# ishine/tts-max

Hardware: AMD Instinct MI355X
Metric: audio-codes/sec + RTF@24kHz, TTS-1 bs=1/32, at 1/2/4/8 MI355X (higher is better)
Workload: dtype bf16; 1 GPU; tts1 bf16 bs=1/GPU: prompt 202 tokens (150 codes), 500 greedy codes, codec codec-24k on 650 codes; model=TTS-1 (Llama-3.2-1B dims, V=193856, tied) + xcodec2-style codec codec-24k, global_batch=1, seq_len=702, parallelism=dp1

## Files before the change

### tts-max_amd/csrc/lm_attn.hip

```cpp
#include <stdexcept>

#include "hip_common.h"
#include "lm_kernels.h"
#include "lm_attn_core.h"

namespace tts {

template <int D>
TTS_DEV float rope_at(const bf16_t* v, int d, const bf16_t* cosr, const bf16_t* sinr) {
  constexpr int H2 = D / 2;
  return rope_elem(v[d], v[d < H2 ? d + H2 : d - H2], d < H2, bf2f(cosr[d]), bf2f(sinr[d]));
}

template <int D>
__global__ __launch_bounds__(256) void rope_append_kernel(AttnArgs a) {
  constexpr int VLD = 8 * D + 8;
  __shared__ __attribute__((aligned(16))) bf16_t vs[16 * VLD];
  const int HD = a.H * D, KD = a.KVH * D;
  if ((int)blockIdx.x < a.rows) {
    const int row = blockIdx.x;
    const int slot = a.row_slot[row], pos = a.row_pos[row];
    const bf16_t* base = a.qkv + (size_t)row * a.ld_qkv;
    const bf16_t* cosr = a.rope_cos + (size_t)pos * D;
    const bf16_t* sinr = a.rope_sin + (size_t)pos * D;
    for (int i = threadIdx.x; i < HD + KD; i += blockDim.x) {
      if (i < HD) {
        const int h = i / D, d = i % D;
        a.q_rot[(size_t)row * HD + i] = f2bf(rope_at<D>(base + h * D, d, cosr, sinr));
      } else {
        const int j = i - HD, h = j / D, d = j % D;
        a.kcache[(((size_t)slot * a.KVH + h) * a.max_seq + pos) * D + d] = f2bf(rope_at<D>(base + HD + h * D, d, cosr, sinr));
      }
    }
    return;
  }
  const int4 blk = a.blocks[blockIdx.x - a.rows];
  const int r0 = blk.x, nr = blk.y, slot = blk.z, p0 = blk.w;
  for (int e = threadIdx.x; e < nr * (KD / 8); e += blockDim.x) {
    const int rr = e / (KD / 8), c = e - rr * (KD / 8);
    *(u32x4_t*)(vs + rr * VLD + c * 8) = *(const u32x4_t*)(a.qkv + (size_t)(r0 + rr) * a.ld_qkv + HD + KD + c * 8);
  }
  __syncthreads();
  for (int e = threadIdx.x; e < KD * 16; e += blockDim.x) {
    const int j = e >> 4, pl = e & 15, h = j / D, d = j % D;
    if (pl < nr)
      a.vtcache[((size_t)slot * a.KVH + h) * D * a.max_seq + vt_off(a.max_seq, d, p0 + pl)] = vs[pl * VLD + j];
  }
}

template <int D>
__global__ __launch_bounds__(dec_nw<D>() * 64) void attn_decode_kernel(AttnArgs a) {
  constexpr int PW = dec_pw<D>(), NW = dec_nw<D>();
  using C = DecShape<D, PW>;
  __shared__ __attribute__((aligned(16))) float qs[DEC_G * D];
  __shared__ __attribute__((aligned(16))) bf16_t knew[D];
  __shared__ __attribute__((aligned(16))) bf16_t vnew[D];
  __shared__ __attribute__((aligned(16))) float red[dec_red_floats<D, NW>()];
  const int row = blockIdx.x / a.KVH, kvh = blockIdx.x % a.KVH;
  const int slot = a.row_slot[row], pos = a.row_pos[row], ctx = pos + 1;
  const int tid = threadIdx.x, lane = tid & 63;
  const int wave = __builtin_amdgcn_readfirstlane(tid >> 6);
  const size_t kvbase = ((size_t)slot * a.KVH + kvh) * a.max_seq * D;
  const bf16_t* kc = a.kcache + kvbase;
  const bf16_t* vtc = a.vtcache + kvbase;
  unsigned long long* stp = a.stamps ? a.stamps + 16384 + (size_t)blockIdx.x * 8 : nullptr;
  TTS_STAMP(stp, 0);
  u32x4_t kf[C::MT][C::KS], vf[C::PS][C::DT];
  if (wave * PW < ctx) {
    dec_load_k<D, PW, D == 64>(kc, wave * PW, ctx, lane, kf);
    dec_load_v<D, PW, D == 64>(vtc, a.max_seq, wave * PW, lane, vf);
  }
  const bf16_t* qrow = a.qkv + (size_t)row * a.ld_qkv;
  const bf16_t* cosr = a.rope_cos + (size_t)pos * D;
  const bf16_t* sinr = a.rope_sin + (size_t)pos * D;
  __shared__ __attribute__((aligned(16))) bf16_t raw[DEC_G * D + 2 * D];
  const bf16_t* qsrc = qrow + kvh * DEC_G * D;
  const bf16_t* ksrc = qrow + a.H * D + kvh * D;
  const bf16_t* vsrc = qrow + a.H * D + a.KVH * D + kvh * D;
  if (a.qkv_part) {
    for (int i = tid; i < DEC_G * D + 2 * D; i += NW * 64) {
      const int col = i < DEC_G * D ? kvh * DEC_G * D + i
                    : (i < DEC_G * D + D ? a.H * D + kvh * D + i - DEC_G * D
                                         : a.H * D + a.KVH * D + kvh * D + i - DEC_G * D - D);
      float v = 0.f;
      for (int sl = 0; sl < a.qkv_nsl; ++sl) v += a.qkv_part[((size_t)sl * a.rows + row) * a.ld_qkv + col];
      raw[i] = f2bf(v);
    }
    lds_barrier();
    qsrc = raw;
    ksrc = raw + DEC_G * D;
    vsrc = raw + DEC_G * D + D;
  }
  for (int i = tid; i < DEC_G * D + D; i += NW * 64) {
    if (i < DEC_G * D) {
      const int g = i / D, d = i % D;
      qs[i] = rope_at<D>(qsrc + g * D, d, cosr, sinr);
    } else {
      const int d = i - DEC_G * D;
      knew[d] = f2bf(rope_at<D>(ksrc, d, cosr, sinr));
      vnew[d] = vsrc[d];
    }
  }
  lds_barrier();
  TTS_STAMP(stp, 2);
  dec_attend<D, PW, NW, D == 64>(kc, vtc, a.max_seq, ctx, a.scale, qs, knew, vnew, red, kf, vf,
                              a.out + (size_t)row * a.H * D + kvh * DEC_G * D);
  TTS_STAMP(stp, 3);
  if (tid < D) {
    a.kcache[kvbase + (size_t)pos * D + tid] = knew[tid];
    a.vtcache[kvbase + vt_off(a.max_seq, tid, pos)] = vnew[tid];
  }
}

void launch_attn_decode_step(const AttnArgs& a, hipStream_t s) {
  if (dry_record(a.D == 64 ? "attn_decode_kernel<64>" : "attn_decode_kernel<128>")) return;
  const dim3 grid(a.rows * a.KVH);
  if (a.D == 64) hipLaunchKernelGGL((attn_decode_kernel<64>), grid, dim3(dec_nw<64>() * 64), 0, s, a);
  else hipLaunchKernelGGL((attn_decode_kernel<128>), grid, dim3(dec_nw<128>() * 64), 0, s, a);
}

template <int D>
__global__ __launch_bounds__(256) void attn_prefill_kernel(AttnArgs a) {
  using C = DecShape<D, 32>;
  const int4 blk = a.blocks[blockIdx.x / a.KVH];
  const int kvh = blockIdx.x % a.KVH;
  const int row0 = blk.x, nrows = blk.y, slot = blk.z, pos0 = blk.w;
  const int tid = threadIdx.x, lane = tid & 63;
  const int h = kvh * DEC_G + __builtin_amdgcn_readfirstlane(tid >> 6);
  const int c = lane & 15, g = lane >> 4;
  const int qpos = pos0 + c;
  const int qrow = row0 + min(c, nrows - 1);
  const size_t kvbase = ((size_t)slot * a.KVH + kvh) * a.max_seq * D;
  const bf16_t* kc = a.kcache + kvbase;
  const bf16_t* vtc = a.vtcache + kvbase;
  const int kend = pos0 + nrows;
  const int nkb = (kend + 31) / 32;
  bf16x8_t qb[C::KS];
#pragma unroll
  for (int ks = 0; ks < C::KS; ++ks)
    qb[ks] = __builtin_bit_cast(bf16x8_t, *(const u32x4_t*)(a.q_rot + (size_t)qrow * a.H * D + h * D + 32 * ks + 8 * g));
  auto scores = [&](int kb, f32x4_t (&s)[2]) {
    u32x4_t kf[2][C::KS];
#pragma unroll
    for (int mt = 0; mt < 2; ++mt) {
      const int p = min(dec_pos(kb * 32, mt, c), kend - 1);
#pragma unroll
      for (int ks = 0; ks < C::KS; ++ks) kf[mt][ks] = *(const u32x4_t*)(kc + (size_t)p * D + 32 * ks + 8 * g);
    }
#pragma unroll
    for (int mt = 0; mt < 2; ++mt) {
      f32x4_t acc = {0.f, 0.f, 0.f, 0.f};
#pragma unroll
      for (int ks = 0; ks < C::KS; ++ks)
        acc = __builtin_amdgcn_mfma_f32_16x16x32_bf16(__builtin_bit_cast(bf16x8_t, kf[mt][ks]), qb[ks], acc, 0, 0, 0);
#pragma unroll
      for (int r = 0; r < 4; ++r) acc[r] = (dec_pos(kb * 32, mt, 4 * g + r) <= qpos) ? acc[r] * a.scale : -INFINITY;
      s[mt] = acc;
    }
  };
  float mx = -INFINITY;
  for (int kb = 0; kb < nkb; ++kb) {
    f32x4_t s[2];
    scores(kb, s);
#pragma unroll
    for (int mt = 0; mt < 2; ++mt)
#pragma unroll
      for (int r = 0; r < 4; ++r) mx = fmaxf(mx, s[mt][r]);
  }
  mx = fmaxf(mx, __shfl_xor(mx, 16, 64));
  mx = fmaxf(mx, __shfl_xor(mx, 32, 64));
  float lsum = 0.f;
  f32x4_t o[C::DT];
#pragma unroll
  for (int dt = 0; dt < C::DT; ++dt) o[dt] = f32x4_t{0.f, 0.f, 0.f, 0.f};
  for (int kb = 0; kb < nkb; ++kb) {
    u32x4_t vf[1][C::DT];
    const int p0 = kb * 32 + 8 * g;
#pragma unroll
    for (int dt = 0; dt < C::DT; ++dt) vf[0][dt] = *(const u32x4_t*)(vtc + vt_off(a.max_seq, 16 * dt + c, p0));
// ... 35 lines not shown
```

### tts-max_amd/csrc/lm_attn_core.h

```cpp
#pragma once
#include "hip_common.h"

namespace tts {

template <int D, int PW>
struct DecShape {
  static constexpr int MT = PW / 16;
  static constexpr int KS = D / 32;
  static constexpr int PS = PW / 32;
  static constexpr int DT = D / 16;
};

constexpr int DEC_G = 4;
constexpr int DEC_NW = 16;
template <int D> constexpr int dec_nw() { return 16; }
template <int D> constexpr int dec_pw() { return D == 64 ? 64 : 32; }

TTS_DEV int vt_off(int S, int d, int p) {
  return (((d >> 4) * (S >> 5) + (p >> 5)) * 16 + (d & 15)) * 32 + (p & 31);
}

TTS_DEV int dec_pos(int base, int mt, int row) {
  return base + 32 * (mt >> 1) + 8 * (row >> 2) + 4 * (mt & 1) + (row & 3);
}

template <int D, int PW, bool O32 = false>
TTS_DEV void dec_load_k(const bf16_t* kc, int base, int ctx, int lane,
                        u32x4_t (&kf)[DecShape<D, PW>::MT][DecShape<D, PW>::KS]) {
  using C = DecShape<D, PW>;
  const int c = lane & 15, g = lane >> 4;
#pragma unroll
  for (int mt = 0; mt < C::MT; ++mt) {
    const int p = min(dec_pos(base, mt, c), ctx - 1);
#pragma unroll
    for (int ks = 0; ks < C::KS; ++ks)
      kf[mt][ks] = O32 ? *(const u32x4_t*)(kc + (p * D + 32 * ks + 8 * g))
                       : *(const u32x4_t*)(kc + (size_t)p * D + 32 * ks + 8 * g);
  }
}
template <int D, int PW, bool O32 = false>
TTS_DEV void dec_load_v(const bf16_t* vtc, int S, int base, int lane,
                        u32x4_t (&vf)[DecShape<D, PW>::PS][DecShape<D, PW>::DT]) {
  using C = DecShape<D, PW>;
  const int c = lane & 15, g = lane >> 4;
#pragma unroll
  for (int ps = 0; ps < C::PS; ++ps) {
    const int pb = min((base >> 5) + ps, (S >> 5) - 1);
    const int o0 = (pb * 16 + c) * 32 + 8 * g;
#pragma unroll
    for (int dt = 0; dt < C::DT; ++dt)
      vf[ps][dt] = O32 ? *(const u32x4_t*)(vtc + (o0 + dt * 16 * S)) : *(const u32x4_t*)(vtc + o0 + (size_t)dt * 16 * S);
  }
}

TTS_DEV uint32_t bits_sel(uint32_t mask, uint32_t a, uint32_t b) { return (a & mask) | (b & ~mask); }
template <int D, int PW>
TTS_DEV void dec_patch_k(int base, int ctx, int lane, const bf16_t* knew,
                         u32x4_t (&kf)[DecShape<D, PW>::MT][DecShape<D, PW>::KS]) {
  using C = DecShape<D, PW>;
  const int c = lane & 15, g = lane >> 4, pn = ctx - 1;
  u32x4_t kn[C::KS];
#pragma unroll
  for (int ks = 0; ks < C::KS; ++ks) kn[ks] = *(const u32x4_t*)(knew + 32 * ks + 8 * g);
#pragma unroll
  for (int mt = 0; mt < C::MT; ++mt) {
    const uint32_t m = dec_pos(base, mt, c) == pn ? 0xffffffffu : 0u;
#pragma unroll
    for (int ks = 0; ks < C::KS; ++ks)
#pragma unroll
      for (int q = 0; q < 4; ++q) kf[mt][ks][q] = bits_sel(m, kn[ks][q], kf[mt][ks][q]);
  }
}
template <int D, int PW>
TTS_DEV void dec_patch_v(int base, int ctx, int lane, const bf16_t* vnew,
                         u32x4_t (&vf)[DecShape<D, PW>::PS][DecShape<D, PW>::DT]) {
  using C = DecShape<D, PW>;
  const int c = lane & 15, g = lane >> 4, pn = ctx - 1;
  uint32_t vn[C::DT];
#pragma unroll
  for (int dt = 0; dt < C::DT; ++dt) vn[dt] = vnew[16 * dt + c];
#pragma unroll
  for (int ps = 0; ps < C::PS; ++ps) {
    const int p0 = base + 32 * ps + 8 * g;
    uint32_t keep[4], put[4];
#pragma unroll
    for (int e2 = 0; e2 < 4; ++e2) {
      const int pl = p0 + 2 * e2, ph = pl + 1;
      keep[e2] = (pl < pn ? 0x0000ffffu : 0u) | (ph < pn ? 0xffff0000u : 0u);
      put[e2] = (pl == pn ? 0x0000ffffu : 0u) | (ph == pn ? 0xffff0000u : 0u);
    }
#pragma unroll
    for (int dt = 0; dt < C::DT; ++dt) {
      const uint32_t nv = vn[dt] | (vn[dt] << 16);
#pragma unroll
      for (int e2 = 0; e2 < 4; ++e2) vf[ps][dt][e2] = (vf[ps][dt][e2] & keep[e2]) | (nv & put[e2]);
    }
  }
}

template <int D>
TTS_DEV bf16x8_t dec_qfrag(const float* qs, int lane, int ks) {
  const int h = (lane & 15) & 3, g = lane >> 4;
  const float4 a = *(const float4*)(qs + h * D + 32 * ks + 8 * g);
  const float4 b = *(const float4*)(qs + h * D + 32 * ks + 8 * g + 4);
  const u32x4_t w = {pack_bf2(a.x, a.y), pack_bf2(a.z, a.w), pack_bf2(b.x, b.y), pack_bf2(b.z, b.w)};
  return __builtin_bit_cast(bf16x8_t, w);
}

template <int D, int PW>
TTS_DEV void dec_scores(const u32x4_t (&kf)[DecShape<D, PW>::MT][DecShape<D, PW>::KS], const float* qs,
                        int base, int ctx, float scale, int lane, f32x4_t (&s)[DecShape<D, PW>::MT]) {
  using C = DecShape<D, PW>;
  const int g = lane >> 4;
#pragma unroll
  for (int mt = 0; mt < C::MT; ++mt) s[mt] = f32x4_t{0.f, 0.f, 0.f, 0.f};
#pragma unroll
  for (int ks = 0; ks < C::KS; ++ks) {
    const bf16x8_t qb = dec_qfrag<D>(qs, lane, ks);
#pragma unroll
    for (int mt = 0; mt < C::MT; ++mt)
      s[mt] = __builtin_amdgcn_mfma_f32_16x16x32_bf16(__builtin_bit_cast(bf16x8_t, kf[mt][ks]), qb, s[mt], 0, 0, 0);
  }
#pragma unroll
  for (int mt = 0; mt < C::MT; ++mt)
#pragma unroll
    for (int r = 0; r < 4; ++r) s[mt][r] = (dec_pos(base, mt, 4 * g + r) < ctx) ? s[mt][r] * scale : -INFINITY;
}

template <int D, int PW>
TTS_DEV void dec_pv(float M, float& lsum, f32x4_t (&s)[DecShape<D, PW>::MT],
                    const u32x4_t (&vf)[DecShape<D, PW>::PS][DecShape<D, PW>::DT], f32x4_t (&o)[DecShape<D, PW>::DT]) {
  using C = DecShape<D, PW>;
#pragma unroll
  for (int mt = 0; mt < C::MT; ++mt)
#pragma unroll
    for (int r = 0; r < 4; ++r) {
      const float p = __builtin_amdgcn_exp2f((s[mt][r] - M) * 1.44269504088896341f);
      lsum += p;
      s[mt][r] = p;
    }
#pragma unroll
  for (int ps = 0; ps < C::PS; ++ps) {
    const u32x4_t pw = {pack_bf2(s[2 * ps][0], s[2 * ps][1]), pack_bf2(s[2 * ps][2], s[2 * ps][3]),
                        pack_bf2(s[2 * ps + 1][0], s[2 * ps + 1][1]), pack_bf2(s[2 * ps + 1][2], s[2 * ps + 1][3])};
    const bf16x8_t pb = __builtin_bit_cast(bf16x8_t, pw);
#pragma unroll
    for (int dt = 0; dt < C::DT; ++dt)
      o[dt] = __builtin_amdgcn_mfma_f32_16x16x32_bf16(__builtin_bit_cast(bf16x8_t, vf[ps][dt]), pb, o[dt], 0, 0, 0);
  }
}

template <int D, int NW>
constexpr int dec_red_floats() { return NW * DEC_G * 2 + NW * DEC_G * D; }

template <int D, int PW, int NW, class Bar, bool O32 = false>
TTS_DEV void dec_attend_w(const bf16_t* kc, const bf16_t* vtc, int S, int ctx, float scale, const float* qs,
                          const bf16_t* knew, const bf16_t* vnew, float* red,
                          u32x4_t (&kf0)[DecShape<D, PW>::MT][DecShape<D, PW>::KS],
                          u32x4_t (&vf0)[DecShape<D, PW>::PS][DecShape<D, PW>::DT], bf16_t* out, int wave,
                          int tid, Bar bar, unsigned long long* stp = nullptr, uint64_t* gout = nullptr,
                          uint32_t gtag = 0) {
  using C = DecShape<D, PW>;
  const int lane = tid & 63;
  const int c = lane & 15, g = lane >> 4;
  const int npass = (ctx + NW * PW - 1) / (NW * PW);
  float* mred = red;
  float* lred = red + NW * DEC_G;
  float* ored = lred + NW * DEC_G;
  const int base0 = wave * PW;

  f32x4_t s0[C::MT];
  float mx = -INFINITY;
  if (base0 < ctx) {
    dec_patch_k<D, PW>(base0, ctx, lane, knew, kf0);
    dec_patch_v<D, PW>(base0, ctx, lane, vnew, vf0);
    dec_scores<D, PW>(kf0, qs, base0, ctx, scale, lane, s0);
#pragma unroll
    for (int mt = 0; mt < C::MT; ++mt)
#pragma unroll
      for (int r = 0; r < 4; ++r) mx = fmaxf(mx, s0[mt][r]);
  }
  for (int ps = 1; ps < npass; ++ps) {
    const int base = (ps * NW + wave) * PW;
    if (base >= ctx) break;
    u32x4_t kf[C::MT][C::KS];
    dec_load_k<D, PW, O32>(kc, base, ctx, lane, kf);
    dec_patch_k<D, PW>(base, ctx, lane, knew, kf);
    f32x4_t s[C::MT];
    dec_scores<D, PW>(kf, qs, base, ctx, scale, lane, s);
#pragma unroll
    for (int mt = 0; mt < C::MT; ++mt)
#pragma unroll
      for (int r = 0; r < 4; ++r) mx = fmaxf(mx, s[mt][r]);
  }
  mx = fmaxf(mx, __shfl_xor(mx, 16, 64));
  mx = fmaxf(mx, __shfl_xor(mx, 32, 64));
  if (lane < DEC_G) mred[wave * DEC_G + lane] = mx;
  bar();
  TTS_STAMP(stp, 5);
  float M = -INFINITY;
#pragma unroll
  for (int w = 0; w < NW; ++w) M = fmaxf(M, mred[w * DEC_G + (c & 3)]);

  float lsum = 0.f;
  f32x4_t o[C::DT];
#pragma unroll
  for (int dt = 0; dt < C::DT; ++dt) o[dt] = f32x4_t{0.f, 0.f, 0.f, 0.f};
  if (base0 < ctx) dec_pv<D, PW>(M, lsum, s0, vf0, o);
  for (int ps = 1; ps < npass; ++ps) {
    const int base = (ps * NW + wave) * PW;
    if (base >= ctx) break;
    u32x4_t kf[C::MT][C::KS], vf[C::PS][C::DT];
    dec_load_v<D, PW, O32>(vtc, S, base, lane, vf);
    dec_load_k<D, PW, O32>(kc, base, ctx, lane, kf);
    dec_patch_k<D, PW>(base, ctx, lane, knew, kf);
    f32x4_t s[C::MT];
    dec_scores<D, PW>(kf, qs, base, ctx, scale, lane, s);
    dec_patch_v<D, PW>(base, ctx, lane, vnew, vf);
    dec_pv<D, PW>(M, lsum, s, vf, o);
  }
  lsum += __shfl_xor(lsum, 16, 64);
  lsum += __shfl_xor(lsum, 32, 64);
  if (c < DEC_G) {
#pragma unroll
    for (int dt = 0; dt < C::DT; ++dt)
      *(float4*)(ored + (wave * DEC_G + c) * D + 16 * dt + 4 * g) = make_float4(o[dt][0], o[dt][1], o[dt][2], o[dt][3]);
    if (g == 0) lred[wave * DEC_G + c] = lsum;
  }
  bar();
  TTS_STAMP(stp, 6);
  bf16_t gob = 0;
  for (int i = tid; i < DEC_G * D; i += NW * 64) {
    const int h = i / D, d = i - h * D;
    float v[NW];
#pragma unroll
    for (int w = 0; w < NW; ++w) v[w] = lred[w * DEC_G + h];
    float O = 0.f, L = 0.f;
#pragma unroll
    for (int w = 0; w < NW; ++w) L += v[w];
#pragma unroll
    for (int w = 0; w < NW; ++w) v[w] = ored[(w * DEC_G + h) * D + d];
#pragma unroll
    for (int w = 0; w < NW; ++w) O += v[w];
    const bf16_t ob = f2bf(O / L);
    out[h * D + d] = ob;
    if (gout) gob = ob;
  }
  if (gout) {
    bar();
    if (tid < DEC_G * D) ((bf16_t*)ored)[tid] = gob;
    bar();
    if (tid < DEC_G * D / 2)
      __hip_atomic_store(gout + tid, ((uint64_t)gtag << 32) | ((const uint32_t*)ored)[tid], __ATOMIC_RELAXED,
                         __HIP_MEMORY_SCOPE_AGENT);
  }
}

template <int D, int PW, int NW, bool O32 = false>
TTS_DEV void dec_attend(const bf16_t* kc, const bf16_t* vtc, int S, int ctx, float scale, const float* qs,
                        const bf16_t* knew, const bf16_t* vnew, float* red,
                        u32x4_t (&kf0)[DecShape<D, PW>::MT][DecShape<D, PW>::KS],
                        u32x4_t (&vf0)[DecShape<D, PW>::PS][DecShape<D, PW>::DT], bf16_t* out,
                        unsigned long long* stp = nullptr, uint64_t* gout = nullptr, uint32_t gtag = 0) {
  auto bar = [] { lds_barrier(); };
  dec_attend_w<D, PW, NW, decltype(bar), O32>(kc, vtc, S, ctx, scale, qs, knew, vnew, red, kf0, vf0, out,
                          __builtin_amdgcn_readfirstlane(threadIdx.x >> 6), threadIdx.x, bar, stp, gout, gtag);
}

TTS_DEV float rope_elem(bf16_t x, bf16_t xr, bool lower_half, float c, float sn) {
  const float rot = lower_half ? -bf2f(xr) : bf2f(xr);
  return rbf(rbf(bf2f(x) * c) + rbf(rot * sn));
}

}
```

### tts-max_amd/csrc/lm_gemm_kernel.h

```cpp
#pragma once
#include <algorithm>
#include <cstdio>
#include <stdexcept>
#include <type_traits>

#include "hip_common.h"
#include "lm_kernels.h"
#include "lm_attn_core.h"

namespace tts {

constexpr int wgemm_ea(int waves) { return waves >= 16 ? 1 : (waves >= 8 ? 2 : 4); }
__host__ __device__ inline int wgemm_red_floats(int waves, int ksplit, int ng, int mt, int M, int Kl) {
  const int upw = waves / ksplit;
  int r = upw * (ksplit - 1) * ng * mt * 4 * 64;
  r = r > upw * mt * 16 * 2 ? r : upw * mt * 16 * 2;
  const int segs = (M * (Kl / 8) + 63) / 64;
  r = r > segs ? r : segs;
  r = r > Kl / 2 ? r : Kl / 2;
  return r + 64;
}

constexpr int wgemm_fattn_d(int ku) { return ku == 2 ? 64 : 128; }
template <int D>
constexpr size_t fattn_lds_bytes() {
  return (size_t)DEC_G * D * 4 + (DEC_G * D / 2 + D) * 4 + 2 * D * 2 + (size_t)dec_red_floats<D, DEC_NW>() * 4;
}
template <typename Poll>
TTS_DEV bool fattn_wait(Poll ready, int* err, int spins, bool report) {
  for (int n = 1; !ready(); ++n) {
    if (n > spins) {
      if (report) __hip_atomic_store(err, 1, __ATOMIC_RELAXED, __HIP_MEMORY_SCOPE_AGENT);
      return false;
    }
    if ((n & 511) == 0 && __hip_atomic_load(err, __ATOMIC_RELAXED, __HIP_MEMORY_SCOPE_AGENT)) return false;
    __builtin_amdgcn_s_sleep(1);
  }
  return true;
}

template <int NT, int D>
TTS_DEV void fattn_consumer(const WgemmArgs& wa, char* smem, int b) {
  static_assert(NT == DEC_NW * 64, "the fused attention runs on 16-wave workgroups");
  constexpr int PW = dec_pw<D>(), G = DEC_G, H2 = D / 2;
  using C = DecShape<D, PW>;
  const AttnArgs& a = wa.fa;
  float* qs = (float*)smem;
  uint32_t* raw = (uint32_t*)(qs + G * D);
  const bf16_t* rawb = (const bf16_t*)raw;
  bf16_t* knew = (bf16_t*)(raw + G * D / 2 + D);
  bf16_t* vnew = knew + D;
  float* red = (float*)(vnew + D);
  const int tid = threadIdx.x, lane = tid & 63;
  const int wave = __builtin_amdgcn_readfirstlane(tid >> 6);
  const int row = b / a.KVH, kvh = b % a.KVH;
  const int slot = a.row_slot[row], pos = a.row_pos[row], ctx = pos + 1;
  const size_t kvbase = ((size_t)slot * a.KVH + kvh) * a.max_seq * D;
  const bf16_t* kc = a.kcache + kvbase;
  const bf16_t* vtc = a.vtcache + kvbase;
  unsigned long long* stp = wa.stamps ? wa.stamps + (size_t)blockIdx.x * 32 : nullptr;
  TTS_STAMP(stp, 0);
  u32x4_t kf[C::MT][C::KS], vf[C::PS][C::DT];
  if (wave * PW < ctx) {
    dec_load_k<D, PW>(kc, wave * PW, ctx, lane, kf);
    dec_load_v<D, PW>(vtc, a.max_seq, wave * PW, lane, vf);
  }
  const int qd = tid % D;
  const float qc = bf2f(a.rope_cos[(size_t)pos * D + qd]), qsn = bf2f(a.rope_sin[(size_t)pos * D + qd]);

  const uint32_t tag = ((uint32_t)pos << 6) | (uint32_t)wa.fattn_layer;
  const int nq = G * D / 2, ngr = nq + D;
  if (tid < ngr) {
    int col;
    if (tid < nq) col = kvh * G * D + 2 * tid;
    else if (tid < nq + D / 2) col = a.H * D + kvh * D + 2 * (tid - nq);
    else col = a.H * D + a.KVH * D + kvh * D + 2 * (tid - nq - D / 2);
    const uint64_t* gp = wa.gran + (size_t)row * (a.ld_qkv / 2) + col / 2;
    uint64_t v;
    fattn_wait([&] {
      v = __hip_atomic_load(gp, __ATOMIC_RELAXED, __HIP_MEMORY_SCOPE_AGENT);
      return (uint32_t)(v >> 32) == tag;
    }, wa.fattn_err, wa.fattn_spins, true);
    raw[tid] = (uint32_t)v;
  }
  lds_barrier();
  TTS_STAMP(stp, 1);
  if (tid < G * D) {
    const int g = tid / D;
    qs[tid] = rope_elem(rawb[tid], rawb[g * D + (qd < H2 ? qd + H2 : qd - H2)], qd < H2, qc, qsn);
  } else if (tid < G * D + D) {
    const int d = tid - G * D;
    knew[d] = f2bf(rope_elem(rawb[G * D + d], rawb[G * D + (d < H2 ? d + H2 : d - H2)], d < H2, qc, qsn));
    vnew[d] = rawb[G * D + D + d];
  }
  lds_barrier();
  TTS_STAMP(stp, 2);
  dec_attend<D, PW, DEC_NW>(kc, vtc, a.max_seq, ctx, a.scale, qs, knew, vnew, red, kf, vf,
                            a.out + (size_t)row * a.H * D + kvh * G * D, stp,
                            wa.fo_units ? wa.gran + (size_t)wa.M * (wa.N / 2) + (size_t)row * (a.H * D / 2) + kvh * G * D / 2
                                        : nullptr,
                            tag);
  TTS_STAMP(stp, 3);
  if (tid < D) {
    a.kcache[kvbase + (size_t)pos * D + tid] = knew[tid];
    a.vtcache[kvbase + vt_off(a.max_seq, tid, pos)] = vnew[tid];
  }
}

TTS_DEV bf16x8_t as_bf16x8(u32x4_t v) { return __builtin_bit_cast(bf16x8_t, v); }

template <int KU, int KSPLIT, int R>
TTS_DEV void fused_oproj(const WgemmArgs& a, bf16_t* xs, float* red, int wave, int lane, uint32_t tag, int u) {
  const int kpart = wave % KSPLIT;
  const int nr = min(a.fo_ur, a.fo_units);
  u32x4_t wr[R][KU];
#pragma unroll
  for (int st = 0; st < R; ++st)
#pragma unroll
    for (int kk = 0; kk < KU; ++kk)
      wr[st][kk] = __builtin_nontemporal_load((const u32x4_t*)a.fo_w +
                                              ((((long long)st * nr + u) * KSPLIT + kpart) * KU + kk) * 64 + lane);
  const bf16_t rr = a.fo_resid[u * 16 + (lane & 15)];
  const uint64_t* g = a.gran + a.N / 2 + kpart * 64 + lane;
  uint64_t v;
  fattn_wait([&] {
    v = __hip_atomic_load(g, __ATOMIC_RELAXED, __HIP_MEMORY_SCOPE_AGENT);
    return (bool)__all((uint32_t)(v >> 32) == tag);
  }, a.fattn_err, a.fattn_spins, lane == 0);
  *(uint32_t*)(xs + kpart * 128 + 2 * lane) = (uint32_t)v;
  asm volatile("s_waitcnt lgkmcnt(0)" ::: "memory");
  f32x4_t acc = {0.f, 0.f, 0.f, 0.f};
  const int akoff = 8 * (lane >> 4);
#pragma unroll
  for (int st = 0; st < R; ++st)
#pragma unroll
    for (int kk = 0; kk < KU; ++kk) {
      const int k = ((kpart * R + st) * KU + kk) * 32 + akoff;
      const u32x4_t av = *(const u32x4_t*)(xs + k);
      acc = __builtin_amdgcn_mfma_f32_16x16x32_bf16(as_bf16x8(av), as_bf16x8(wr[st][kk]), acc, 0, 0, 0);
    }
  if (kpart > 0) *(f32x4_t*)(red + ((size_t)(kpart - 1) * 64 + lane) * 4) = acc;
  lds_barrier();
  if (kpart == 0) {
    constexpr int HB = 8;
#pragma unroll
    for (int p0 = 1; p0 < KSPLIT; p0 += HB) {
      f32x4_t pv[HB];
#pragma unroll
      for (int j = 0; j < HB; ++j)
        if (p0 + j < KSPLIT) pv[j] = *(const f32x4_t*)(red + ((size_t)(p0 + j - 1) * 64 + lane) * 4);
#pragma unroll
      for (int j = 0; j < HB; ++j)
        if (p0 + j < KSPLIT) acc += pv[j];
    }
    if (lane < 16) a.fo_resid[u * 16 + lane] = f2bf(bf2f(rr) + rbf(acc[0]));
  }
}

template <int KU, int KSPLIT, int R>
TTS_DEV void fused_oproj_rows(const WgemmArgs& a, bf16_t* xs, float* red, int wave, int lane, int u) {
  const int M = a.M, HD = a.fa.H * a.fa.D, ldxs = HD + 8, hid = a.fo_units * 16;
  unsigned long long* stp = a.stamps ? a.stamps + (size_t)blockIdx.x * 32 : nullptr;
  TTS_STAMP(stp, 0);
  const int kpart = wave % KSPLIT;
  const int nr = min(a.fo_ur, a.fo_units);
  const int KTc = (HD >> 5) / a.fo_kc, kt_pc = KTc / KSPLIT, Sc = kt_pc / KU;
  auto ktile = [&](int st, int kk) {
    const int ch = st / Sc;
    return ch * KTc + kpart * kt_pc + (st - ch * Sc) * KU + kk;
  };
  u32x4_t wr[R][KU];
#pragma unroll
  for (int st = 0; st < R; ++st)
#pragma unroll
    for (int kk = 0; kk < KU; ++kk)
      wr[st][kk] = __builtin_nontemporal_load((const u32x4_t*)a.fo_w +
                                              ((((long long)st * nr + u) * KSPLIT + kpart) * KU + kk) * 64 + lane);
  bf16_t rr[4];
#pragma unroll
  for (int r = 0; r < 4; ++r) rr[r] = a.fo_resid[(size_t)min(4 * (lane >> 4) + r, M - 1) * hid + u * 16 + (lane & 15)];
// ... 743 lines not shown
```

### tts-max_amd/csrc/lm_head_screen.hip

```cpp
#include <math.h>

#include "hip_common.h"
#include "lm_kernels.h"

namespace tts {

typedef __attribute__((ext_vector_type(4))) int i32x4_t;

namespace {

constexpr int kScrWaves = 4;
constexpr int kScrKU = 8;
constexpr int kScrR = 2;

TTS_DEV float f_up(double d) {
  float f = (float)d;
  if ((double)f < d) f = nextafterf(f, INFINITY);
  return f;
}
TTS_DEV double wave_sum_f64(double v) {
#pragma unroll
  for (int o = 32; o > 0; o >>= 1) v += __shfl_xor(v, o, 64);
  return v;
}
// ... 243 lines not shown
  int nu = 0;
  for (int u = gw; u < units; u += ur, ++nu) {
    int aoff = 0;
    if constexpr (MT * KT8 > 32) asm volatile("" : "+v"(aoff));
    const int c = u * 16 + col;
    const float4 cs = a.cst[c];
    uint32_t sw[MT][2];
#pragma unroll
    for (int mt = 0; mt < MT; ++mt)
#pragma unroll
      for (int p = 0; p < 2; ++p) sw[mt][p] = a.seen[(size_t)min(8 * mt + 2 * g4 + p, M - 1) * a.seen_stride + (c >> 5)];
    i32x4_t acc[MT];
#pragma unroll
    for (int mt = 0; mt < MT; ++mt) acc[mt] = i32x4_t{0, 0, 0, 0};
#pragma unroll
    for (int st = 0; st < S; st += R) {
#pragma unroll
      for (int j = 0; j < R; ++j) {
#pragma unroll
        for (int kk = 0; kk < KU; ++kk) {
          const int kb = (st + j) * KU + kk;
#pragma unroll
          for (int mt = 0; mt < MT; ++mt) {
            if constexpr (kScrProbe & 1) {
              acc[mt][0] ^= (int)wr[j][kk][0];
            } else {
              const i32x4_t af = *(const i32x4_t*)(Al + aoff + (16 * mt + col) * ldA + kb * 64 + 16 * g4);
              acc[mt] = __builtin_amdgcn_mfma_i32_16x16x64_i8(af, __builtin_bit_cast(i32x4_t, wr[j][kk]), acc[mt], 0, 0, 0);
            }
          }
        }
        issue(wr[j]);
      }
    }
#pragma unroll
    for (int mt = 0; mt < MT; ++mt)
#pragma unroll
      for (int p = 0; p < 2; ++p) {
        const int m = 8 * mt + 2 * g4 + p;
        float ub = -INFINITY;
        if (kScrProbe & 2) {
          if (acc[mt][0] == 12345) a.part_val[0] = 0.f;
          continue;
        }
        if (m < M) {
          const float hq = (float)acc[mt][2 * p], lq = (float)acc[mt][2 * p + 1];
          const float Sf = fmaf(hq, 256.f, lq);
          const float av = Sf * rsx[m] * cs.x;
          const float e = fmaf(rnx[m], fmaf(gam, cs.z, cs.y), rndx[m] * cs.w) * (1.f + 0x1p-20f) +
                          (fabsf(av) + fmaf(fabsf(hq), 256.f, fabsf(lq)) * rsx[m] * cs.x) * 0x1p-21f + 1e-30f;
          const uint16_t* crow = a.counts ? a.counts + (size_t)m * a.seen_stride * 32 : nullptr;
          ub = head_proc_bound<true>(rbf(av + e), sw[mt][p], c, a.penalty, inv_pen, crow, a.freq_penalty, eosr[mt][p]);
          const float lb =
              head_proc_bound<false>(rbf(av - e), sw[mt][p], c, a.penalty, inv_pen, crow, a.freq_penalty, eosr[mt][p]);
          if (a.ub) a.ub[(size_t)m * a.ldu + c] = ub;
          lbm[mt][p] = fmaxf(lbm[mt][p], lb);
        }
        ub = row16_max(ub);
        if (col == 0 && nu < kScrMaxUPW) umx[(wave * kScrMaxUPW + nu) * MMAX + m] = ub;
      }
  }

#pragma unroll
  for (int mt = 0; mt < MT; ++mt)
#pragma unroll
    for (int p = 0; p < 2; ++p) {
#pragma unroll
      for (int o = 1; o < 16; o <<= 1) lbm[mt][p] = fmaxf(lbm[mt][p], __shfl_xor(lbm[mt][p], o, 64));
      if (col == 0) rlb[wave * MMAX + 8 * mt + 2 * g4 + p] = lbm[mt][p];
    }
  if (tid == 0) *ntl = 0;
  if (a.check) __threadfence();
  __syncthreads();
  const unsigned long long ep = (unsigned long long)*a.epoch;
  const int shard = blockIdx.x & 7;
  if (tid < M) {
    float v = rlb[tid];
#pragma unroll
    for (int w = 1; w < kScrWaves; ++w) v = fmaxf(v, rlb[w * MMAX + tid]);
    const unsigned long long mine = (ep << 32) | f2key(v);
    const unsigned long long old =
        __hip_atomic_fetch_max(a.lbg + tid * 8 + shard, mine, __ATOMIC_RELAXED, __HIP_MEMORY_SCOPE_AGENT);
    const unsigned long long cur = old > mine ? old : mine;
    LBc[tid] = key2f((uint32_t)cur);
  }
  __syncthreads();
  if (a.spins > 0 && tid < 64) {
    const uint32_t per = gridDim.x >> 3;
    uint32_t target = 0;
    if (tid == 0) {
      const uint32_t old = __hip_atomic_fetch_add(a.arrive + shard * 16, 1u, __ATOMIC_RELAXED, __HIP_MEMORY_SCOPE_AGENT);
      target = (old / per + 1) * per;
    }
    target = __shfl(target, 0, 64);
    const uint32_t* ctr = a.arrive + (lane & 7) * 16;
    for (int n = 0; n < a.spins; ++n) {
      const bool ok = __hip_atomic_load(ctr, __ATOMIC_RELAXED, __HIP_MEMORY_SCOPE_AGENT) - target < 0x80000000u;
      if (__all(ok)) break;
      __builtin_amdgcn_s_sleep(1);
    }
  }
  __syncthreads();
  if (tid < M * 8) {
    const int m = tid >> 3;
    const unsigned long long cur = __hip_atomic_load(a.lbg + tid, __ATOMIC_RELAXED, __HIP_MEMORY_SCOPE_AGENT);
    float v = (cur >> 32) == ep ? key2f((uint32_t)cur) : -INFINITY;
#pragma unroll
    for (int o = 1; o < 8; o <<= 1) v = fmaxf(v, __shfl_xor(v, o, 64));
    if ((tid & 7) == 0) LBc[m] = fmaxf(LBc[m], v);
  }
  __syncthreads();
  if (tid < kScrWaves * kScrMaxUPW) {
    const int w = tid / kScrMaxUPW, i = tid % kScrMaxUPW;
    const int u = (blockIdx.x * kScrWaves + w) + i * ur;
    bool f = false;
    if (u < units) {
      if (a.check) f = true;
      for (int m = 0; m < M; ++m) f = f || umx[(w * kScrMaxUPW + i) * MMAX + m] >= LBc[m];
    }
    if (f) tl[atomicAdd(ntl, 1)] = u;
  }
  __syncthreads();

  constexpr int KT = K / 32, KTW = KT / kScrWaves;
  const int nflag = (a.diag & 1) ? 0 : *ntl;
  if ((a.diag & 2) && tid == 0) atomicAdd(a.err + 2, *ntl);
  float bv[MTB][4];
  int bi[MTB][4];
#pragma unroll
  for (int mb = 0; mb < MTB; ++mb)
#pragma unroll
    for (int r = 0; r < 4; ++r) { bv[mb][r] = -INFINITY; bi[mb][r] = 0x7fffffff; }
  auto load = [&](u32x4_t (&wf)[KTW], int t) {
#pragma unroll
    for (int j = 0; j < KTW; ++j) {
      const int kt = wave * KTW + j;
      const int KTc = KT / a.hkc, ch = kt / KTc, ki = kt - ch * KTc;
      const int st = ch * (KTc / a.hku) + ki / a.hku, kk = ki % a.hku;
      const int rr = t / a.hur, ui = t - rr * a.hur, nr = min(units - rr * a.hur, a.hur);
      const int tile = rr * a.hur * KT + (st * nr + ui) * a.hku + kk;
      wf[j] = __builtin_nontemporal_load((const u32x4_t*)a.w + (size_t)tile * 64 + lane);
    }
  };
  u32x4_t axg[PRE ? MTB : 1][PRE ? KTW : 1];
  if constexpr (PRE) {
#pragma unroll
    for (int mb = 0; mb < MTB; ++mb)
#pragma unroll
      for (int j = 0; j < KTW; ++j)
        axg[mb][j] = *(const u32x4_t*)(a.x + (size_t)min(16 * mb + col, M - 1) * a.ldx + (wave * KTW + j) * 32 + 8 * g4);
  }
  const bf16_t* xrow = Xl + (size_t)min(col, M - 1) * ldX + 8 * g4;
  auto chain = [&](const u32x4_t (&wf)[KTW], int t) {
    f32x4_t acc4[MTB];
#pragma unroll
    for (int mb = 0; mb < MTB; ++mb) acc4[mb] = f32x4_t{0.f, 0.f, 0.f, 0.f};
#pragma unroll
    for (int s = 0; s < kScrWaves; ++s) {
      if (wave == s) {
#pragma unroll
        for (int mb = 0; mb < MTB; ++mb)
          if (s > 0) acc4[mb] = xacc[mb * 64 + lane];
#pragma unroll
        for (int j = 0; j < KTW; ++j)
#pragma unroll
          for (int mb = 0; mb < MTB; ++mb) {
            u32x4_t av;
// ... 141 lines not shown
```

Measured before the change: 1704 audio-codes/s.

## Store decode Q in bf16 LDS, skip non-tail K/V patching, register-shuffle RoPE

```diff
diff --git a/tts-max_amd/csrc/lm_attn.hip b/tts-max_amd/csrc/lm_attn.hip
--- a/tts-max_amd/csrc/lm_attn.hip
+++ b/tts-max_amd/csrc/lm_attn.hip
@@ -52,7 +52,7 @@
 __global__ __launch_bounds__(dec_nw<D>() * 64) void attn_decode_kernel(AttnArgs a) {
   constexpr int PW = dec_pw<D>(), NW = dec_nw<D>();
   using C = DecShape<D, PW>;
-  __shared__ __attribute__((aligned(16))) float qs[DEC_G * D];
+  __shared__ __attribute__((aligned(16))) bf16_t qs[DEC_G * D];
   __shared__ __attribute__((aligned(16))) bf16_t knew[D];
   __shared__ __attribute__((aligned(16))) bf16_t vnew[D];
   __shared__ __attribute__((aligned(16))) float red[dec_red_floats<D, NW>()];
@@ -94,7 +94,7 @@
   for (int i = tid; i < DEC_G * D + D; i += NW * 64) {
     if (i < DEC_G * D) {
       const int g = i / D, d = i % D;
-      qs[i] = rope_at<D>(qsrc + g * D, d, cosr, sinr);
+      qs[i] = f2bf(rope_at<D>(qsrc + g * D, d, cosr, sinr));
     } else {
       const int d = i - DEC_G * D;
       knew[d] = f2bf(rope_at<D>(ksrc, d, cosr, sinr));
diff --git a/tts-max_amd/csrc/lm_attn_core.h b/tts-max_amd/csrc/lm_attn_core.h
--- a/tts-max_amd/csrc/lm_attn_core.h
+++ b/tts-max_amd/csrc/lm_attn_core.h
@@ -54,21 +54,23 @@
 }
 
 TTS_DEV uint32_t bits_sel(uint32_t mask, uint32_t a, uint32_t b) { return (a & mask) | (b & ~mask); }
+template <int PW>
+TTS_DEV bool dec_tail(int base, int ctx) { return __builtin_amdgcn_readfirstlane(base + PW > ctx - 1) != 0; }
 template <int D, int PW>
 TTS_DEV void dec_patch_k(int base, int ctx, int lane, const bf16_t* knew,
                          u32x4_t (&kf)[DecShape<D, PW>::MT][DecShape<D, PW>::KS]) {
   using C = DecShape<D, PW>;
   const int c = lane & 15, g = lane >> 4, pn = ctx - 1;
-  u32x4_t kn[C::KS];
-#pragma unroll
-  for (int ks = 0; ks < C::KS; ++ks) kn[ks] = *(const u32x4_t*)(knew + 32 * ks + 8 * g);
-#pragma unroll
-  for (int mt = 0; mt < C::MT; ++mt) {
-    const uint32_t m = dec_pos(base, mt, c) == pn ? 0xffffffffu : 0u;
-#pragma unroll
-    for (int ks = 0; ks < C::KS; ++ks)
-#pragma unroll
-      for (int q = 0; q < 4; ++q) kf[mt][ks][q] = bits_sel(m, kn[ks][q], kf[mt][ks][q]);
+  uint32_t m[C::MT];
+#pragma unroll
+  for (int mt = 0; mt < C::MT; ++mt) m[mt] = dec_pos(base, mt, c) == pn ? 0xffffffffu : 0u;
+#pragma unroll
+  for (int ks = 0; ks < C::KS; ++ks) {
+    const u32x4_t kn = *(const u32x4_t*)(knew + 32 * ks + 8 * g);
+#pragma unroll
+    for (int mt = 0; mt < C::MT; ++mt)
+#pragma unroll
+      for (int q = 0; q < 4; ++q) kf[mt][ks][q] = bits_sel(m[mt], kn[q], kf[mt][ks][q]);
   }
 }
 template <int D, int PW>
@@ -99,17 +101,14 @@
 }
 
 template <int D>
-TTS_DEV bf16x8_t dec_qfrag(const float* qs, int lane, int ks) {
+TTS_DEV bf16x8_t dec_qfrag(const bf16_t* qs, int lane, int ks) {
   const int h = (lane & 15) & 3, g = lane >> 4;
-  const float4 a = *(const float4*)(qs + h * D + 32 * ks + 8 * g);
-  const float4 b = *(const float4*)(qs + h * D + 32 * ks + 8 * g + 4);
-  const u32x4_t w = {pack_bf2(a.x, a.y), pack_bf2(a.z, a.w), pack_bf2(b.x, b.y), pack_bf2(b.z, b.w)};
-  return __builtin_bit_cast(bf16x8_t, w);
-}
-
-template <int D, int PW>
-TTS_DEV void dec_scores(const u32x4_t (&kf)[DecShape<D, PW>::MT][DecShape<D, PW>::KS], const float* qs,
-                        int base, int ctx, float scale, int lane, f32x4_t (&s)[DecShape<D, PW>::MT]) {
+  return __builtin_bit_cast(bf16x8_t, *(const u32x4_t*)(qs + h * D + 32 * ks + 8 * g));
+}
+
+template <int D, int PW>
+TTS_DEV void dec_scores(const u32x4_t (&kf)[DecShape<D, PW>::MT][DecShape<D, PW>::KS], const bf16_t* qs,
+                        int base, int ctx, float scale, int lane, bool tail, f32x4_t (&s)[DecShape<D, PW>::MT]) {
   using C = DecShape<D, PW>;
   const int g = lane >> 4;
 #pragma unroll
@@ -124,7 +123,16 @@
 #pragma unroll
   for (int mt = 0; mt < C::MT; ++mt)
 #pragma unroll
-    for (int r = 0; r < 4; ++r) s[mt][r] = (dec_pos(base, mt, 4 * g + r) < ctx) ? s[mt][r] * scale : -INFINITY;
+    for (int r = 0; r < 4; ++r) s[mt][r] *= scale;
+  __builtin_amdgcn_sched_barrier(0);
+  if (tail) {
+#pragma unroll
+    for (int mt = 0; mt < C::MT; ++mt)
+#pragma unroll
+      for (int r = 0; r < 4; ++r) s[mt][r] = (dec_pos(base, mt, 4 * g + r) < ctx) ? s[mt][r] : -INFINITY;
+    __builtin_amdgcn_sched_barrier(0);
+  }
+  __builtin_amdgcn_sched_barrier(0);
 }
 
 template <int D, int PW>
@@ -154,7 +162,7 @@
 constexpr int dec_red_floats() { return NW * DEC_G * 2 + NW * DEC_G * D; }
 
 template <int D, int PW, int NW, class Bar, bool O32 = false>
-TTS_DEV void dec_attend_w(const bf16_t* kc, const bf16_t* vtc, int S, int ctx, float scale, const float* qs,
+TTS_DEV void dec_attend_w(const bf16_t* kc, const bf16_t* vtc, int S, int ctx, float scale, const bf16_t* qs,
                           const bf16_t* knew, const bf16_t* vnew, float* red,
                           u32x4_t (&kf0)[DecShape<D, PW>::MT][DecShape<D, PW>::KS],
                           u32x4_t (&vf0)[DecShape<D, PW>::PS][DecShape<D, PW>::DT], bf16_t* out, int wave,
@@ -171,10 +179,15 @@
 
   f32x4_t s0[C::MT];
   float mx = -INFINITY;
+  const bool tail0 = dec_tail<PW>(base0, ctx);
   if (base0 < ctx) {
-    dec_patch_k<D, PW>(base0, ctx, lane, knew, kf0);
-    dec_patch_v<D, PW>(base0, ctx, lane, vnew, vf0);
-    dec_scores<D, PW>(kf0, qs, base0, ctx, scale, lane, s0);
+    __builtin_amdgcn_sched_barrier(0);
+    if (tail0) {
+      dec_patch_k<D, PW>(base0, ctx, lane, knew, kf0);
+      __builtin_amdgcn_sched_barrier(0);
+    }
+    __builtin_amdgcn_sched_barrier(0);
+    dec_scores<D, PW>(kf0, qs, base0, ctx, scale, lane, tail0, s0);
 #pragma unroll
     for (int mt = 0; mt < C::MT; ++mt)
 #pragma unroll
@@ -185,9 +198,15 @@
     if (base >= ctx) break;
     u32x4_t kf[C::MT][C::KS];
     dec_load_k<D, PW, O32>(kc, base, ctx, lane, kf);
-    dec_patch_k<D, PW>(base, ctx, lane, knew, kf);
+    const bool tail = dec_tail<PW>(base, ctx);
+    __builtin_amdgcn_sched_barrier(0);
+    if (tail) {
+      dec_patch_k<D, PW>(base, ctx, lane, knew, kf);
+      __builtin_amdgcn_sched_barrier(0);
+    }
+    __builtin_amdgcn_sched_barrier(0);
     f32x4_t s[C::MT];
-    dec_scores<D, PW>(kf, qs, base, ctx, scale, lane, s);
+    dec_scores<D, PW>(kf, qs, base, ctx, scale, lane, tail, s);
 #pragma unroll
     for (int mt = 0; mt < C::MT; ++mt)
 #pragma unroll
@@ -196,6 +215,12 @@
   mx = fmaxf(mx, __shfl_xor(mx, 16, 64));
   mx = fmaxf(mx, __shfl_xor(mx, 32, 64));
   if (lane < DEC_G) mred[wave * DEC_G + lane] = mx;
+  __builtin_amdgcn_sched_barrier(0);
+  if (base0 < ctx && tail0) {
+    dec_patch_v<D, PW>(base0, ctx, lane, vnew, vf0);
+    __builtin_amdgcn_sched_barrier(0);
+  }
+  __builtin_amdgcn_sched_barrier(0);
   bar();
   TTS_STAMP(stp, 5);
   float M = -INFINITY;
@@ -213,10 +238,20 @@
     u32x4_t kf[C::MT][C::KS], vf[C::PS][C::DT];
     dec_load_v<D, PW, O32>(vtc, S, base, lane, vf);
     dec_load_k<D, PW, O32>(kc, base, ctx, lane, kf);
-    dec_patch_k<D, PW>(base, ctx, lane, knew, kf);
+    const bool tail = dec_tail<PW>(base, ctx);
+    __builtin_amdgcn_sched_barrier(0);
+    if (tail) {
+      dec_patch_k<D, PW>(base, ctx, lane, knew, kf);
+      __builtin_amdgcn_sched_barrier(0);
+    }
+    __builtin_amdgcn_sched_barrier(0);
     f32x4_t s[C::MT];
-    dec_scores<D, PW>(kf, qs, base, ctx, scale, lane, s);
-    dec_patch_v<D, PW>(base, ctx, lane, vnew, vf);
+    dec_scores<D, PW>(kf, qs, base, ctx, scale, lane, tail, s);
+    if (tail) {
+      dec_patch_v<D, PW>(base, ctx, lane, vnew, vf);
+      __builtin_amdgcn_sched_barrier(0);
+    }
+    __builtin_amdgcn_sched_barrier(0);
     dec_pv<D, PW>(M, lsum, s, vf, o);
   }
   lsum += __shfl_xor(lsum, 16, 64);
@@ -229,6 +264,7 @@
   }
   bar();
   TTS_STAMP(stp, 6);
+  static_assert(DEC_G * D <= NW * 64, "one output element per thread");
   bf16_t gob = 0;
   for (int i = tid; i < DEC_G * D; i += NW * 64) {
     const int h = i / D, d = i - h * D;
@@ -247,17 +283,15 @@
     if (gout) gob = ob;
   }
   if (gout) {
-    bar();
-    if (tid < DEC_G * D) ((bf16_t*)ored)[tid] = gob;
-    bar();
-    if (tid < DEC_G * D / 2)
-      __hip_atomic_store(gout + tid, ((uint64_t)gtag << 32) | ((const uint32_t*)ored)[tid], __ATOMIC_RELAXED,
+    const uint32_t nb = (uint32_t)__builtin_amdgcn_update_dpp(0, (int)gob, 0xB1, 0xf, 0xf, false);
+    if (tid < DEC_G * D && !(tid & 1))
+      __hip_atomic_store(gout + (tid >> 1), ((uint64_t)gtag << 32) | (nb << 16) | gob, __ATOMIC_RELAXED,
                          __HIP_MEMORY_SCOPE_AGENT);
   }
 }
 
 template <int D, int PW, int NW, bool O32 = false>
-TTS_DEV void dec_attend(const bf16_t* kc, const bf16_t* vtc, int S, int ctx, float scale, const float* qs,
+TTS_DEV void dec_attend(const bf16_t* kc, const bf16_t* vtc, int S, int ctx, float scale, const bf16_t* qs,
                         const bf16_t* knew, const bf16_t* vnew, float* red,
                         u32x4_t (&kf0)[DecShape<D, PW>::MT][DecShape<D, PW>::KS],
                         u32x4_t (&vf0)[DecShape<D, PW>::PS][DecShape<D, PW>::DT], bf16_t* out,
diff --git a/tts-max_amd/csrc/lm_gemm_kernel.h b/tts-max_amd/csrc/lm_gemm_kernel.h
--- a/tts-max_amd/csrc/lm_gemm_kernel.h
+++ b/tts-max_amd/csrc/lm_gemm_kernel.h
@@ -24,7 +24,7 @@
 constexpr int wgemm_fattn_d(int ku) { return ku == 2 ? 64 : 128; }
 template <int D>
 constexpr size_t fattn_lds_bytes() {
-  return (size_t)DEC_G * D * 4 + (DEC_G * D / 2 + D) * 4 + 2 * D * 2 + (size_t)dec_red_floats<D, DEC_NW>() * 4;
+  return (size_t)(DEC_G * D + 2 * D) * 2 + (size_t)dec_red_floats<D, DEC_NW>() * 4;
 }
 template <typename Poll>
 TTS_DEV bool fattn_wait(Poll ready, int* err, int spins, bool report) {
@@ -45,10 +45,8 @@
   constexpr int PW = dec_pw<D>(), G = DEC_G, H2 = D / 2;
   using C = DecShape<D, PW>;
   const AttnArgs& a = wa.fa;
-  float* qs = (float*)smem;
-  uint32_t* raw = (uint32_t*)(qs + G * D);
-  const bf16_t* rawb = (const bf16_t*)raw;
-  bf16_t* knew = (bf16_t*)(raw + G * D / 2 + D);
+  bf16_t* qs = (bf16_t*)smem;
+  bf16_t* knew = qs + G * D;
   bf16_t* vnew = knew + D;
   float* red = (float*)(vnew + D);
   const int tid = threadIdx.x, lane = tid & 63;
@@ -62,14 +60,16 @@
   TTS_STAMP(stp, 0);
   u32x4_t kf[C::MT][C::KS], vf[C::PS][C::DT];
   if (wave * PW < ctx) {
-    dec_load_k<D, PW>(kc, wave * PW, ctx, lane, kf);
-    dec_load_v<D, PW>(vtc, a.max_seq, wave * PW, lane, vf);
-  }
-  const int qd = tid % D;
-  const float qc = bf2f(a.rope_cos[(size_t)pos * D + qd]), qsn = bf2f(a.rope_sin[(size_t)pos * D + qd]);
+    dec_load_k<D, PW, D == 128>(kc, wave * PW, ctx, lane, kf);
+    dec_load_v<D, PW, D == 128>(vtc, a.max_seq, wave * PW, lane, vf);
+  }
+  const int qd = (2 * tid) % D;
+  const uint32_t cs2 = *(const uint32_t*)(a.rope_cos + (size_t)pos * D + qd);
+  const uint32_t sn2 = *(const uint32_t*)(a.rope_sin + (size_t)pos * D + qd);
 
   const uint32_t tag = ((uint32_t)pos << 6) | (uint32_t)wa.fattn_layer;
   const int nq = G * D / 2, ngr = nq + D;
+  uint32_t raw = 0;
   if (tid < ngr) {
     int col;
     if (tid < nq) col = kvh * G * D + 2 * tid;
@@ -81,21 +81,25 @@
       v = __hip_atomic_load(gp, __ATOMIC_RELAXED, __HIP_MEMORY_SCOPE_AGENT);
       return (uint32_t)(v >> 32) == tag;
     }, wa.fattn_err, wa.fattn_spins, true);
-    raw[tid] = (uint32_t)v;
-  }
+    raw = (uint32_t)v;
+  }
+#ifdef TTS_STAMPS
   lds_barrier();
+#endif
   TTS_STAMP(stp, 1);
-  if (tid < G * D) {
-    const int g = tid / D;
-    qs[tid] = rope_elem(rawb[tid], rawb[g * D + (qd < H2 ? qd + H2 : qd - H2)], qd < H2, qc, qsn);
-  } else if (tid < G * D + D) {
-    const int d = tid - G * D;
-    knew[d] = f2bf(rope_elem(rawb[G * D + d], rawb[G * D + (d < H2 ? d + H2 : d - H2)], d < H2, qc, qsn));
-    vnew[d] = rawb[G * D + D + d];
+  const uint32_t rawr = (uint32_t)__shfl_xor((int)raw, D / 4, 64);
+  if (tid < ngr) {
+    uint32_t w = raw;
+    if (tid < nq + D / 2) {
+      const bool lower = qd < H2;
+      w = pack_bf2(rope_elem((bf16_t)raw, (bf16_t)rawr, lower, bf_lo(cs2), bf_lo(sn2)),
+                   rope_elem((bf16_t)(raw >> 16), (bf16_t)(rawr >> 16), lower, bf_hi(cs2), bf_hi(sn2)));
+    }
+    ((uint32_t*)qs)[tid] = w;
   }
   lds_barrier();
   TTS_STAMP(stp, 2);
-  dec_attend<D, PW, DEC_NW>(kc, vtc, a.max_seq, ctx, a.scale, qs, knew, vnew, red, kf, vf,
+  dec_attend<D, PW, DEC_NW, D == 128>(kc, vtc, a.max_seq, ctx, a.scale, qs, knew, vnew, red, kf, vf,
                             a.out + (size_t)row * a.H * D + kvh * G * D, stp,
                             wa.fo_units ? wa.gran + (size_t)wa.M * (wa.N / 2) + (size_t)row * (a.H * D / 2) + kvh * G * D / 2
                                         : nullptr,
diff --git a/tts-max_amd/csrc/lm_head_screen.hip b/tts-max_amd/csrc/lm_head_screen.hip
--- a/tts-max_amd/csrc/lm_head_screen.hip
+++ b/tts-max_amd/csrc/lm_head_screen.hip
@@ -349,7 +349,7 @@
     const unsigned long long old =
         __hip_atomic_fetch_max(a.lbg + tid * 8 + shard, mine, __ATOMIC_RELAXED, __HIP_MEMORY_SCOPE_AGENT);
     const unsigned long long cur = old > mine ? old : mine;
-    LBc[tid] = key2f((uint32_t)cur);
+    LBc[tid] = (cur >> 32) == ep ? key2f((uint32_t)cur) : v;
   }
   __syncthreads();
   if (a.spins > 0 && tid < 64) {
```

New measurement: 1738 audio-codes/s, median of 6. 1.02x the previous value.
